# jsh58/Genrich

Measured on AMD Instinct MI355X. Metric: genome bases p-scored/sec, hg38 50M frags, higher is better.
Workload: dtype int32 pileup (1/120 units) + f64 p-values; 1 GPU; hg38 25 contigs (3088286401 bp), 50000000 paired fragments x 1 replicate(s), treatment only, -p 0.01 (BASELINE.json configs[1]); parallelism=chromosome-sharded x1, collectives=none, rccl_nranks=0, intervals=83948696, tables_written_in_step=none: the sweep walks the loose (end, V) slots, p = table p(V)

## Files before the change

genrich_amd/csrc/gx_api.hip:

```cpp
#include "gx_host_ctx.h"
#include "gx_host_coll.h"
#include "gx_host_build.h"
#include "gx_host_sweep.h"
#include "gx_host_stats.h"
#include "gx_host_count.h"
#include "gx_host_regions.h"



extern "C" {

const char* gx_strerror(int status) {
  switch (status) {
    case GX_OK: return "";
    case GX_ERR_MEM: return "Cannot allocate memory";
    case GX_ERR_GEN: return "No analyzable genome (length=0)";
    case GX_ERR_EXPT: return "Experimental sample has no analyzable fragments";
    case GX_ERR_PILE: return "Invalid pileup value (< 0)";
    case GX_ERR_POS: return ": read aligned beyond reference end";
    case GX_ERR_ALNS: return "Disallowed number of alignments";
    case GX_ERR_ARR: return "Failure creating experimental pileup";
    case GX_ERR_PVAL: return "Failure collecting p-values";
    case GX_ERR_DF: return "Invalid df in pchisq()";
    case GX_ERR_ORDER: return "API called out of order";
// ... 38 lines not shown
  memset(ctx->riskHost.p, 0, 32);
  HIPCHECK(hipMemsetAsync(ctx->dRisk.p, 0, 32, ctx->stream));
  HIPCHECK(hipMemsetAsync(ctx->dDeep.p, 0, sizeof(DeepTab), ctx->stream));
  HIPCHECK(hipMemsetAsync(ctx->misc.p, 0, M_WORDS * 4, ctx->stream));
  HIPCHECK(hipMemsetAsync(ctx->dScal.p, 0, sizeof(Scalars), ctx->stream));
  HIPCHECK(hipMemsetAsync(ctx->dStatus.p, 0, 64, ctx->stream));
  HIPCHECK(hipFuncSetAttribute(reinterpret_cast<const void*>(k_tile<true, false>),
                               hipFuncAttributeMaxDynamicSharedMemorySize, TL_LDS * 4));
  {
    hipDeviceProp_t prop;
    HIPCHECK(hipGetDeviceProperties(&prop, ctx->device));
    ctx->numCU = prop.multiProcessorCount;
    int nb = 0;
    HIPCHECK(hipOccupancyMaxActiveBlocksPerMultiprocessor(&nb, k_tile<true, false>, TL_NT, TL_LDS * 4));
    ctx->resTile = std::max(1, nb) * ctx->numCU;
    HIPCHECK(hipOccupancyMaxActiveBlocksPerMultiprocessor(&nb, k_tile<true, true>, TL_NT, TL_LDS_HALF * 4));
    ctx->resTileHalf = std::max(1, nb) * ctx->numCU;
    HIPCHECK(hipOccupancyMaxActiveBlocksPerMultiprocessor(&nb, k_tile_fast, 64, 0));
    ctx->resTileFast = std::max(1, std::min(nb, TF_WG_PER_CU)) * ctx->numCU;
    if (ctx->knob.debug)
      fprintf(stderr, "k_tile workgroups: half %d, wide %d, fast %d\n", ctx->resTileHalf, ctx->resTile, ctx->resTileFast);
    HIPCHECK(hipOccupancyMaxActiveBlocksPerMultiprocessor(&nb, k_scan_iv, STL_NT, 0));
    ctx->resSweep = std::max(1, std::min(nb, 4)) * ctx->numCU;
  }
  HIPCHECK(hipStreamSynchronize(ctx->stream));
  return GX_OK;
}

void gx_destroy(gx_ctx* ctx) {
  if (!ctx) return;
  (void)hipSetDevice(ctx->device);
  if (ctx->stream) (void)hipStreamSynchronize(ctx->stream);
  if (ctx->comm) {
    if (const gxrccl::Api* api = gxrccl::load(nullptr)) (void)api->commDestroy(ctx->comm);
    ctx->comm = nullptr;
  }
  for (auto& ph : ctx->phases) {
    (void)hipEventDestroy(ph.a);
    (void)hipEventDestroy(ph.b);
  }
  if (ctx->stream) (void)hipStreamDestroy(ctx->stream);
  if (ctx->side) (void)hipStreamDestroy(ctx->side);
  if (ctx->sideEv) (void)hipEventDestroy(ctx->sideEv);
  for (hipEvent_t e : ctx->evPool) (void)hipEventDestroy(e);
  for (hipEvent_t e : ctx->stageFree) if (e) (void)hipEventDestroy(e);
  delete ctx;
// ... 745 lines not shown
```

genrich_amd/csrc/gx_host_build.h:

```cpp
#pragma once
namespace {

uint64_t genome_len_for(const gx_ctx* ctx, const std::vector<uint8_t>& present) {
  uint64_t g = 0;
  for (u32 i = 0; i < ctx->nChrom; i++)
    if (!ctx->skip[i] && present[i]) {
      g += ctx->len[i];
      for (size_t j = 0; j + 1 < ctx->bed[i].size(); j += 2) g -= ctx->bed[i][j + 1] - ctx->bed[i][j];
    }
  return g;
}

int upload_chroms(gx_ctx* ctx, bool force = true) {
  bool changed = force;
  for (u32 i = 0; i < ctx->nChrom; i++) {
    const u32 f = (ctx->skip[i] ? CH_SKIP : 0) | (ctx->save[i] ? CH_SAVE : 0) | (ctx->owned[i] ? CH_OWNED : 0);
    changed |= f != ctx->hChrom[i].flags;
    ctx->hChrom[i].flags = f;
  }
  if (!changed) return GX_OK;
  HIPCHECK(hipMemcpyAsync(ctx->dChrom.p, ctx->hChrom.data(), ctx->nChrom * sizeof(DChrom), hipMemcpyHostToDevice,
                          ctx->stream));
  return GX_OK;
}
// ... 11 lines not shown
  return GX_OK;
}

int flush_begin(gx_ctx* ctx) {
  if (!ctx->beginPending) return GX_OK;
  hipLaunchKernelGGL(k_begin_sample, dim3(1), dim3(64), 0, ctx->stream, ctx->dScal.as<Scalars>(), ctx->beginGenome);
  ctx->beginPending = false;
  return GX_OK;
}

int stash_or_pack(gx_ctx* ctx, Pileup& P) {
  if (ctx->hasBed) return pack_pileup(ctx, P);
  if (P.inLoose) return GX_OK;
  recycle(ctx, P.looseEnd);
  recycle(ctx, P.looseV);
  recycle(ctx, P.meta);
  P.looseEnd = std::move(ctx->looseEnd);
  P.looseV = std::move(ctx->looseV);
  P.meta = std::move(ctx->tileMeta);
  P.inLoose = true;
  return GX_OK;
}

template <typename Segs> static u32 class_chunks(const Segs& segs) {
  u32 best = 0;
  for (u32 x = 0; x < (u32)NXCD; x++) {
    u32 c = 0;
    for (auto& sg : segs) {
      const u32 b = (u32)((sg.n + S2_CHUNK - 1) / S2_CHUNK);
      c += b / NXCD + (b % NXCD > x ? 1u : 0u);
    }
    best = std::max(best, c);
  }
  return best;
}

int unpack_segs(gx_ctx* ctx, bool all) {
  size_t total = 0;
  auto wanted = [&](const gx_ctx::Seg& sg) {
    return sg.packed && sg.n && (all || (reinterpret_cast<uintptr_t>(sg.p) & 15u) || (!sg.ready && (sg.n & 1u)));
  };
  for (auto& sg : ctx->segs)
    if (wanted(sg)) total += sg.n;
  if (!total) return GX_OK;
  if (ctx->unpackUsed == ctx->unpackBufs.size()) ctx->unpackBufs.emplace_back();
  DevBuf& buf = ctx->unpackBufs[ctx->unpackUsed++];
  HIPCHECK(buf.ensure(total * sizeof(gx_event)));
  hipStream_t s = ctx->stream;
  gx_event* at = buf.as<gx_event>();
  for (auto& sg : ctx->segs) {
    if (!wanted(sg)) continue;
    if (sg.ready) HIPCHECK(hipStreamWaitEvent(s, sg.ready, 0));
    hipLaunchKernelGGL(k_unpack_events, dim3((u32)std::min<size_t>((sg.n + 255) / 256, 8192)), dim3(256), 0, s,
                       reinterpret_cast<const uint2*>(sg.p), sg.n, reinterpret_cast<uint4*>(at));
    sg.p = at;
    sg.ready = nullptr;
    sg.packed = false;
// ... 26 lines not shown
  const bool pairsAllowed = !K.noPairs;
  const bool fracOk = pairsAllowed && !K.noFracPairs;
  const bool fracLikely = ctx->sawFrac || ctx->fracHint;
  const bool fused = P.fused =
      !backoff && unit32 && (!ctx->hasBed || (pairsAllowed && !K.noBedFused && !fracLikely)) && ctx->sbShift <= SBT_MAXSHIFT && !noFused &&
      (!fracLikely || fracOk) && !ctx->fusedOff && !forceSlowFrag && (size_t)nEv <= (size_t)std::max(1u, nL1base) * 64000 &&
      (size_t)2 * nEv + nTiles + ctx->nBedEdges + 64 < ((size_t)1 << 30);
  P.pairs = fused && !reuseSort && pairsAllowed;
  P.fracPairs = P.pairs && fracLikely;
  int sbS = ctx->sbShift;
  u32 nL1 = nL1base;
  const bool forceHalf = K.forceHalfBins != 0;
  if (P.pairs && (!P.fracPairs || forceHalf || K.fracHalfBins) && sbS > 0 &&
      (forceHalf || (size_t)2 * nEv > (size_t)std::max(1u, nL1base) * (SBT_KEYCAP - SBT_KEYCAP / 10)) &&
      ((nTiles + (1u << (sbS - 1)) - 1) >> (sbS - 1)) <= (u32)MAX_BINS_P && !K.noHalfBins) {
    sbS--;
    nL1 = (nTiles + (1u << sbS) - 1) >> sbS;
  }
  P.sbS = sbS, P.nL1 = nL1;
  P.jmax = ctx->ptJmax;
  P.poolPages[0] = P.poolPages[1] = (u32)(nEv >> PgCfg<u32>::SHIFT) + NXCD * nL1 + 4;
  P.poolPages[2] = (u32)(((size_t)2 * nEv) >> PgCfg<u64>::SHIFT) + NXCD * nL1 + 4;
  P.nCoarse = (std::max(1u, nL1) + (1u << s2_fine_shift(nL1)) - 1) >> s2_fine_shift(nL1);
  P.jmaxC = class_chunks(ctx->segs) + 3;
  for (auto& sg : ctx->segs) P.nWG1 += (u32)((sg.n + S2_CHUNK - 1) / S2_CHUNK);
  P.wantEarly = !isCtrl && (!P.multiRank || P.earlyColl) && !ctx->par.qval_opt && !ctx->hasBed && unit32 && !noLoose && !forceSlowFrag &&
                !ctx->sawFrac;
  const bool qLooseMay = ctx->par.qval_opt && !K.noQLoose && !ctx->qLooseBad && !ctx->sawFrac && !ctx->fracHint && !K.noPackHist;
  P.wantLate = !P.wantEarly && !isCtrl && !P.multiRank && (!ctx->par.qval_opt || qLooseMay) && !ctx->hasBed && unit32 && !noLoose &&
               !K.noLateLoose && fused && !forceSlowFrag;
  P.closeInScan = P.wantEarly && !P.multiRank;
  P.looseCap = (size_t)2 * nEv + nTiles + ctx->nBedEdges + 16;
  P.ivCap = (size_t)2 * nEv + ctx->nChrom + ctx->nBedEdges + 16;
  P.tChunks = (nTiles + STL_CHUNK - 1) / STL_CHUNK;
  P.fragFused = !ctx->hasBed && (!fused || P.fracPairs);
  P.dense = P.pairs && (size_t)2 * nEv > (size_t)std::max(1u, nL1) * (SBT_KEYCAP - SBT_KEYCAP / 16);
  if (P.dense) {
    const size_t want = (size_t)2 * nEv / std::max(1u, nL1);
    auto rounds = [&](u32 tr) { return (want + sbt_keycap(tr) - 1) / sbt_keycap(tr); };
    P.denseSmall = rounds((u32)SBT_TR_DENSE) < rounds((u32)SBT_TR);
    if (K.sbtTr) P.denseSmall = K.sbtTr == SBT_TR_DENSE;
  }
  return GX_OK;
}

PagedStream paged(const gx_ctx* ctx, const BuildPlan& P, int q) {
  const gx_ctx::Stream& st = ctx->str[q];
// ... 89 lines not shown
  HIPCHECK(hipMemsetAsync(ctx->looseCtl.p, 0, ctx->looseCtl.cap, s));
  HIPCHECK(hipMemsetAsync(&ctx->fragSum.as<FragFix>()->nList, 0, 12, s));
  HIPCHECK(hipMemsetAsync(nw_word(ctx, NW_WIDE), 0, 4, s));
  HIPCHECK(hipMemsetAsync(nw_word(ctx, NW_HEAVY), 0, 4, s));
  return GX_OK;
}

int sort_level1(gx_ctx* ctx, const BuildPlan& P) {
  hipStream_t s = ctx->stream;
  FragFix* ff = ctx->fragSum.as<FragFix>();
  if ((ctx->hasBed && !P.fused) || !P.unit32 || ctx->knob.forceSlowFrag) HIPCHECK(hipMemsetAsync(&ff->slow, 1, 4, s));
  if (P.reuseSort) return dbg_sync(ctx, "k_sort1");
  const PagedStream PG0 = paged(ctx, P, 0), PG1 = paged(ctx, P, 1), PG2 = paged(ctx, P, 2);
  const Sort1Out so1{ff->fragSum, &ff->slow, ctx->endAtLen.as<u32>(), nw_word(ctx, NW_HOT)};
  const u32 nListsC = NXCD * P.nCoarse;
  const PagedStream PC{ctx->poolC.p, ctx->ptC.as<u32>(), ctx->curC.as<u32>(), ctx->curC.as<u32>() + nListsC, P.jmaxC, P.nWG1 + 2 * nListsC + 8, nListsC};
  static constexpr decltype(&k_sort_a<false, false>) SORT_A[2][2] = {{k_sort_a<false, false>, k_sort_a<false, true>},
                                                                     {k_sort_a<true, false>, k_sort_a<true, true>}};
  for (auto& seg : ctx->segs) {
    if (!seg.n) continue;
    if (seg.ready) HIPCHECK(hipStreamWaitEvent(s, seg.ready, 0));
    const u32 blocks = (u32)((seg.n + S1_CHUNK - 1) / S1_CHUNK);
    if (P.pairs) {
      hipLaunchKernelGGL(SORT_A[P.fracPairs][seg.packed], dim3(blocks), dim3(S2_NT), 0, s, seg.p, (u32)seg.n, ctx->dChrom.as<DChrom>(), ctx->nChrom, P.sbS,
                         P.nL1, P.nCoarse, PC, ctx->auxC.as<uint8_t>(), PG2, ctx->binNet.as<int>(), so1, ctx->dStatus.as<u32>());
      ctx->packedUsed |= seg.packed;
    } else
      hipLaunchKernelGGL(P.unit32 ? k_sort1<true> : k_sort1<false>, dim3(blocks), dim3(S1_NT), 0, s, seg.p, (u32)seg.n,
                         ctx->dChrom.as<DChrom>(), ctx->nChrom, P.sbS, P.nL1, PG0, PG1, PG2, so1, ctx->dStatus.as<u32>());
  }
  if (P.pairs && P.nEv)
    hipLaunchKernelGGL(k_sort_b, dim3(NXCD * (P.jmaxC - 3 + P.nCoarse)), dim3(S2_NT), 0, s, PC, (const uint8_t*)ctx->auxC.as<uint8_t>(),
                       P.nCoarse, P.nL1, PG0, ctx->dStatus.as<u32>());
  return dbg_sync(ctx, "k_sort1");
}

long long* early_words(const gx_ctx* ctx, const BuildPlan& P) { return P.earlyColl ? ctx->dColl.as<long long>() + 4 : nullptr; }
int early_allreduce(gx_ctx* ctx, const BuildPlan& P) {
  if (!P.earlyColl) return GX_OK;
  hipLaunchKernelGGL(k_early_words, dim3(1), dim3(64), 0, ctx->stream, ctx->fragSum.as<FragFix>(), P.wantEarly ? 0 : 1, early_words(ctx, P));
  if (int rc__ = allreduce_words(ctx, early_words(ctx, P), 3)) return rc__;
  ctx->earlyOwed = false;
  return GX_OK;
}

int scan_bins(gx_ctx* ctx, const BuildPlan& P) {
  gx_ctx::Stream* S = ctx->str;
  auto capOf = [&](int shift) -> u32 { return P.jmax >= (1u << (31 - shift)) ? 0x7FFFFFFFu : P.jmax << shift; };
  BinScan bs{{S[0].cursor.as<u32>(), S[1].cursor.as<u32>(), S[2].cursor.as<u32>()},
             {capOf(PgCfg<u32>::SHIFT), capOf(PgCfg<u32>::SHIFT), capOf(PgCfg<u64>::SHIFT)},
             {S[0].sbOff.as<u32>(), S[1].sbOff.as<u32>(), S[2].sbOff.as<u32>()},
             ctx->endAtLen.as<u32>(), ctx->chromW0.as<int>(), ctx->nChrom, ctx->fragSum.as<FragFix>(), ctx->dScal.as<Scalars>(), ctx->looseCtl.as<LooseCtl>(),
             P.wantEarly ? 1 : 0, P.pairs ? 1 : 0, ctx->binNet.as<int>(), nw_word(ctx, NW_NEED_PAGES), early_words(ctx, P)};
  static_assert(PV_LUT % 1024 == 0, "k_bins_lut: four of k_pval_lut's workgroups per block");
  if (P.wantEarly)
    hipLaunchKernelGGL(k_bins_lut, dim3(4 + PV_LUT / 1024), dim3(1024), 0, ctx->stream, bs, P.nL1, ctx->pvLut.as<float>(),
// ... 429 lines not shown
```

genrich_amd/csrc/gx_host_ctx.h:

```cpp
#pragma once
#include <hip/hip_runtime.h>
#include <rocprim/device/device_radix_sort.hpp>

#include <algorithm>
#include <cmath>
#include <cstdio>
#include <cstdlib>
#include <cstring>
#include <atomic>
#include <chrono>
#include <string>
#include <vector>
#include <unistd.h>

#include "gx_merge.h"
#include "gx_rccl.h"
#include "gx_sort.h"
#include "gx_tile_fast.h"
#include "gx_sbtile.h"
#include "gx_dups.h"
#include "gx_bhx.h"
#include "gx_saturate.h"
#include "gx_count.h"
#include "gx_regions.h"
// ... 119 lines not shown
  int noFracPairs = 0;
  int noBedFused = 0;
  int bhVariant = -1;
  int mergeWg = 0;
  int noQLoose = 0;
  int noLateLoose = 0;
  int noLazyQ = 0;
  int noPackHist = 0;
  int noMergeP = 0;
  int forceHalfBins = 0;
  int noHalfBins = 0;
  int fracHalfBins = 0;
  int noEarlyColl = 0;
  int regWindows = 0;
  int noDenseBh = 0;
  int qtMulti = 0;
  int forceColl = 0;
  int sbShift = -1;
  long long runCapMin = 0;
  int bhCapLog = 0;
  int ptJmax = 0;
  int sbtTr = 0;
  int sbtGrid = 0;
  int roctx = 0;
  int fault = 0;
};
struct BuildPlan {
  int isCtrl = 0;
  bool reuseSort = false;
  u32 nEv = 0;
  bool unit32 = false;
  bool multiRank = false;
  bool earlyColl = false;
  bool fused = false;
  bool pairs = false;
  bool fracPairs = false;
  int sbS = 0;
  u32 nL1 = 0;
  u32 nCoarse = 0, jmaxC = 0, nWG1 = 0;
  u32 jmax = 0;
  u32 poolPages[3] = {0, 0, 0};
  bool wantEarly = false;
  bool wantLate = false;
  bool closeInScan = false;
  bool dense = false;
  bool denseSmall = false;
  bool fragFused = false;
  size_t looseCap = 0, ivCap = 0;
  u32 tChunks = 0;
  bool masks() const { return wantEarly || wantLate; }
};
struct KnobDef { const char* name; int Knobs::*i; long long Knobs::*ll; };
const KnobDef KNOBS[] = {
    {"GX_DEBUG", &Knobs::debug, nullptr}, {"GX_DEBUG_RETRY", &Knobs::debugRetry, nullptr}, {"GX_NO_SPIN", &Knobs::noSpin, nullptr},
    {"GX_FORCE_REC64", &Knobs::forceRec64, nullptr}, {"GX_FORCE_SLOWFRAG", &Knobs::forceSlowFrag, nullptr},
    {"GX_NO_FUSED", &Knobs::noFused, nullptr}, {"GX_NO_LOOSE", &Knobs::noLoose, nullptr}, {"GX_NO_PAIRS", &Knobs::noPairs, nullptr},
    {"GX_NO_FRAC_PAIRS", &Knobs::noFracPairs, nullptr}, {"GX_NO_BED_FUSED", &Knobs::noBedFused, nullptr}, {"GX_NO_MERGE_P", &Knobs::noMergeP, nullptr}, {"GX_NO_PACK_HIST", &Knobs::noPackHist, nullptr}, {"GX_NO_LAZY_Q", &Knobs::noLazyQ, nullptr}, {"GX_NO_LATE_LOOSE", &Knobs::noLateLoose, nullptr}, {"GX_NO_Q_LOOSE", &Knobs::noQLoose, nullptr}, {"GX_MERGE_WG", &Knobs::mergeWg, nullptr}, {"GX_BH_VARIANT", &Knobs::bhVariant, nullptr}, {"GX_FORCE_HALF_BINS", &Knobs::forceHalfBins, nullptr},
    {"GX_NO_HALF_BINS", &Knobs::noHalfBins, nullptr}, {"GX_FRAC_HALF_BINS", &Knobs::fracHalfBins, nullptr}, {"GX_NO_EARLY_COLL", &Knobs::noEarlyColl, nullptr},
    {"GX_NO_DENSE_BH", &Knobs::noDenseBh, nullptr}, {"GX_REG_WINDOWS", &Knobs::regWindows, nullptr}, {"GX_QT_MULTI", &Knobs::qtMulti, nullptr}, {"GX_FORCE_COLL", &Knobs::forceColl, nullptr},
    {"GX_SBSHIFT", &Knobs::sbShift, nullptr}, {"GX_RUN_CAP_MIN", nullptr, &Knobs::runCapMin}, {"GX_BH_CAPLOG", &Knobs::bhCapLog, nullptr},
    {"GX_PT_JMAX", &Knobs::ptJmax, nullptr}, {"GX_FAULT", &Knobs::fault, nullptr}, {"GX_SBT_TR", &Knobs::sbtTr, nullptr}, {"GX_SBT_GRID", &Knobs::sbtGrid, nullptr},
    {"GX_ROCTX", &Knobs::roctx, nullptr},
};
bool set_knob(Knobs& k, const char* name, const char* value) {
  for (const KnobDef& d : KNOBS)
    if (!strcmp(d.name, name)) {
      long long v = 1;
      if (value && *value) {
        char* end = nullptr;
        v = strtoll(value, &end, 10);
        if (end == value) v = 1;
      }
      if (d.i) k.*(d.i) = (int)v; else k.*(d.ll) = v;
      return true;
    }
  return false;
}

}

struct gx_ctx {
  gx_params par{};
  Knobs knob;
  int device = 0;
// ... 92 lines not shown
  PinnedBuf hPeaks;
  size_t nHostPeaks = 0;
  u32* nIvTarget = nullptr;
  PinnedBuf mailBuf;
  HostMail* mail = nullptr;
  uint64_t genomeLenUsed = 0, peakBP = 0;
  int rank = 0, world = 1;
  gx_allreduce_i64_fn allreduce = nullptr;
  void* user = nullptr;
  ncclComm_t comm = nullptr;
  bool forceColl = false;
  DevBuf bigBins;
  DevBuf dColl, dCounts, dGather, bhDense, bhxSmall, bhxRecv, bhxKeys, bhxLens, bhxQ, bhxOut, bhxAns;
  bool rangeBhUsed = false;
  bool denseBhUsed = false;
  int phaseLevel = 0;
  std::string phaseFilter = "tile";
  u32 mailSeq = 0;
  u32 statusSeen = 1;
  u64 runCap = 0, runSeen = 0;
  bool phaseOpen = false;
  bool roctxOpen = false;
  int numCU = 0, resTile = 0, resTileHalf = 0, resTileFast = 0, resSweep = 0;
  std::vector<DevBuf> pool;
  struct KeptSample {
    int rep = 0;
    bool ctrl = false;
    std::vector<Seg> segs;
    std::vector<uint8_t> save;
    std::vector<DevBuf> chunks, unpacks;
    DevBuf sat;
  };
  bool countOn = false;
  bool peaksReady = false;
  bool countsReady = false;
  std::vector<KeptSample> kept;
  u32 cntPk = 0;
  DevBuf cntIn, cntIdx, cntDiff, cntRes;
  PinnedBuf cntStage, cntHost;
  bool cntLdsSet = false;
  bool regionsReady = false;
  size_t regN = 0;
  u32 regSamples = 0;
  u32 regInvCap = 1u << 14;
  DevBuf regIn, regIdx, regHist, regSums, regRes, regInv;
  PinnedBuf regStage, regHost;
// ... 236 lines not shown
```

genrich_amd/csrc/gx_sort.h:

```cpp
#pragma once
#include "gx_kernels.h"
#include "gx_stats.h"

namespace gx {

constexpr u32 ST_PT_FULL = 512u;
constexpr u32 ST_SB_FULL = 1024u;
constexpr u32 ST_SB_FRAC = 2048u;

template <typename R> struct PgCfg { static constexpr int SHIFT = 12; };
template <> struct PgCfg<u32> { static constexpr int SHIFT = 13; };
constexpr u32 PG_BYTES = 32768;

struct PagedStream {
  void* pool;
  u32* pt;
  u32* cursor;
  u32* pagesUsed;
  u32 jmax, poolPages;
  u32 nLists;
};

__device__ __forceinline__ u32 first_page(u32 list) { return 1u + list; }

// ... 479 lines not shown
#define GX_S2_BATCH 4
#endif
constexpr int S2_BATCH = GX_S2_BATCH;
constexpr int S2_LCHROM = 96;
constexpr int S2_ITEMS = 8192 / S2_NT;
static_assert(S2_ITEMS == 16 || S2_ITEMS == 8, "512 or 1024 threads");
constexpr int S2_CHUNK = S2_NT * S2_ITEMS;
constexpr int S2_KEYS = 128;
constexpr int MAX_BINS_P = 8192;
__host__ __device__ inline int s2_fine_shift(u32 nBins) { return nBins > 4096u ? 7 : 6; }
static_assert(S2_CHUNK == (1 << PgCfg<u32>::SHIFT), "k_sort_b: one workgroup per page of a coarse list");
static_assert(S2_CHUNK == S1_CHUNK, "one grid size for the level-1 kernels");

struct S2Lds {
  u32 cnt[S2_KEYS];
  __attribute__((aligned(16))) uint4 run[S2_KEYS];
  u32 total;
  u32 wtot[2];
  u32 scratch[24];
  u32 stage[S2_CHUNK];
  uint16_t ka[S2_CHUNK];
};

template <bool AUX, int KEYS>
__device__ __forceinline__ void scatter64(const u32 (&rec)[S2_ITEMS], u32 (&ka)[S2_ITEMS], const PagedStream& P,
                                          uint8_t* __restrict__ auxPool, u32 listBase, u32 nKeys, S2Lds& L, u32* __restrict__ st) {
  static_assert(KEYS == 64 || KEYS == 128, "one or two owner wavefronts");
  constexpr int SHIFT = PgCfg<u32>::SHIFT;
  constexpr u32 PG = 1u << SHIFT;
  constexpr u32 KM = (u32)KEYS - 1u;
#pragma unroll
  for (int k = 0; k < S2_ITEMS; k++) ka[k] = (ka[k] & 0xFFFFu) | ((rec[k] != NULL32 ? atomicAdd(&L.cnt[ka[k] & KM], 1u) : 0u) << 16);
  __syncthreads();
  const bool owner = threadIdx.x < (u32)KEYS;
  const u32 key = threadIdx.x;
  u32 c = 0, o = 0, inc = 0, li = 0;
  if (owner) {
    c = key < nKeys ? L.cnt[key] : 0u;
    li = listBase + key;
    if (c) o = atomicAdd(&P.cursor[li], c);
    inc = (u32)dpp_scan_add((int)c);
    if ((key & 63u) == 63u) L.wtot[key >> 6] = inc;
  }
  if (KEYS == 64 && threadIdx.x == 0) L.wtot[1] = 0;
  __syncthreads();
  const u32 in0 = o & (PG - 1), j0 = o >> SHIFT, j1 = (o + c - 1) >> SHIFT;
  u32* row = P.pt + (size_t)li * P.jmax;
  u32 p0 = 0, p1 = 0;
  bool wait0 = false;
  if (owner) {
    if (key == 0) L.total = L.wtot[0] + L.wtot[1];
    if (c) {
      if (j1 != j0) p1 = page_alloc(P, row, j1, st);
      if (j0 == 0)
        p0 = first_page(li);
      else if (in0 == 0)
        p0 = page_alloc(P, row, j0, st);
      else
        wait0 = true;
    }
  }
  __syncthreads();
  if (owner) {
    if (wait0) p0 = page_wait(P, row, j0, st);
    L.run[key] = make_uint4(inc - c + (key >= 64u ? L.wtot[0] : 0u), min(c, PG - in0), (p0 << SHIFT) + in0, p1 << SHIFT);
  }
  __syncthreads();
#pragma unroll
  for (int k = 0; k < S2_ITEMS; k++)
    if (rec[k] != NULL32) {
      const u32 pos = L.run[ka[k] & KM].x + (ka[k] >> 16);
      L.stage[pos] = rec[k];
      L.ka[pos] = (uint16_t)ka[k];
    }
  __syncthreads();
  u32* pool = reinterpret_cast<u32*>(P.pool);
  const u32 cnt = L.total;
#pragma unroll
  for (int h = 0; h < S2_ITEMS; h += 8) {
    u32 v[8], kk[8];
#pragma unroll
    for (int k = 0; k < 8; k++) {
      const u32 i = (u32)(h + k) * S2_NT + threadIdx.x, ii = i < cnt ? i : 0u;
      v[k] = L.stage[ii];
      kk[k] = L.ka[ii];
    }
#pragma unroll
    for (int k = 0; k < 8; k++) {
      const u32 i = (u32)(h + k) * S2_NT + threadIdx.x;
      const uint4 rn = L.run[kk[k] & KM];
      const u32 r = i - rn.x;
      const u32 dst = r < rn.y ? rn.z + r : rn.w + (r - rn.y);
      if (i < cnt) {
        pool[dst] = v[k];
        if (AUX) auxPool[dst] = (uint8_t)(kk[k] >> 8);
      }
    }
  }
}

__device__ __forceinline__ uint4 unpack_event8(u32 start, u32 lcc) {
  return make_uint4(lcc >> 19, start, start + (lcc & 0xFFFFu), (0xA8654321u >> (4u * ((lcc >> 16) & 7u))) & 15u);
}
__global__ __launch_bounds__(256) void k_unpack_events(const uint2* __restrict__ in, size_t n, uint4* __restrict__ out) {
  for (size_t i = (size_t)blockIdx.x * 256 + threadIdx.x; i < n; i += (size_t)gridDim.x * 256) {
    const uint2 e = in[i];
    out[i] = unpack_event8(e.x, e.y);
  }
}

template <bool FRAC, bool PACKED = false>
__global__ __launch_bounds__(S2_NT, GX_S2A_WAVES) void k_sort_a(const gx_event* __restrict__ ev, u32 n, const DChrom* __restrict__ chroms,
                                                     u32 nChrom, int sbShift, u32 nBins, u32 nCoarse, PagedStream PC,
                                                     uint8_t* __restrict__ auxPool, PagedStream PF, int* __restrict__ binNet,
                                                     Sort1Out out, u32* __restrict__ st) {
  __shared__ S2Lds L;
  __shared__ DChrom lchrom[S2_LCHROM];
  const int fineShift = s2_fine_shift(nBins);
  if (!FRAC && (__hip_atomic_load(st, __ATOMIC_RELAXED, __HIP_MEMORY_SCOPE_AGENT) & ST_SB_FRAC)) return;
  const bool chromLds = nChrom <= (u32)S2_LCHROM;
  const u32 x = blockIdx.x % NXCD;
  const u32 begin = blockIdx.x * S2_CHUNK;
  const u32 binMask = (1u << sbShift) - 1u;
  u32 bad = 0, slow = 0, fracSeen = 0;
  u32 covered32 = 0;
  u32 rec[S2_ITEMS], ka[S2_ITEMS];
  if (threadIdx.x < S2_KEYS) L.cnt[threadIdx.x] = 0;
  const uint4* __restrict__ evb = reinterpret_cast<const uint4*>(ev) + begin;
  const u32 lastIn = n - 1u - begin;
#pragma unroll
  for (int k0 = 0; k0 < S2_ITEMS; k0 += S2_BATCH) {
    uint4 e[S2_BATCH];
    bool have[S2_BATCH];
    if constexpr (PACKED) {
      static_assert(S2_BATCH % 2 == 0, "two packed events per 16-byte load");
      const uint4* __restrict__ evp = reinterpret_cast<const uint4*>(reinterpret_cast<const uint2*>(ev) + begin);
#pragma unroll
      for (int q = 0; q < S2_BATCH; q += 2) {
        const u32 lp = ((k0 + q) >> 1) * S2_NT + threadIdx.x;
        have[q] = 2u * lp <= lastIn;
        have[q + 1] = 2u * lp + 1u <= lastIn;
        const uint4 two = evp[min(lp, lastIn >> 1)];
        e[q] = unpack_event8(two.x, two.y);
        e[q + 1] = unpack_event8(two.z, two.w);
      }
    } else {
#pragma unroll
    for (int q = 0; q < S2_BATCH; q++) {
      const u32 li = (k0 + q) * S2_NT + threadIdx.x;
      have[q] = li <= lastIn;
      e[q] = evb[min(li, lastIn)];
    }
    }
    if (k0 == 0) {
      if (chromLds)
        for (u32 i = threadIdx.x; i < nChrom; i += S2_NT) lchrom[i] = chroms[i];
      __syncthreads();
    }
    DChrom cq[S2_BATCH];
    if (chromLds) {
#pragma unroll
      for (int q = 0; q < S2_BATCH; q++) cq[q] = lchrom[min(e[q].x, nChrom - 1)];
    } else {
#pragma unroll
      for (int q = 0; q < S2_BATCH; q++) cq[q] = chroms[min(e[q].x, nChrom - 1)];
    }
#pragma unroll
    for (int q = 0; q < S2_BATCH; q++) {
      const DChrom c = cq[q];
      const u32 cnt = e[q].w;
      const bool cntOk = FRAC ? (cnt <= 10u && ((0x57Eu >> cnt) & 1u)) : cnt == 1u;
      const bool ok1 = have[q] && cntOk && e[q].x < nChrom;
      const bool act = chrom_active(c);
      const u32 len = e[q].z - e[q].y;
      const u32 t0 = c.tileBase + (e[q].y >> TB), t1 = c.tileBase + (e[q].z >> TB);
      const u32 bin = t0 >> sbShift;
      constexpr u32 LENB = FRAC ? 9u : PAIR_LEN_BITS;
      const bool fast = ok1 && act && e[q].z < c.len && len - 1u < (1u << LENB) - 1u && e[q].y < e[q].z && (t1 >> sbShift) == bin;
      const bool nothing = !have[q] || (ok1 && !act);
      const u32 cls = FRAC ? (u32)((0x70605432100ull >> (4u * (cnt & 15u))) & 7ull) << 9 : 0u;
      fracSeen |= (u32)(FRAC && fast && cnt != 1u);
      rec[k0 + q] = fast ? ((((t0 & binMask) << TB) | (e[q].y & (TILE - 1))) << PAIR_LEN_BITS) | cls | len : NULL32;
      ka[k0 + q] = (bin >> fineShift) | ((bin & ((1u << fineShift) - 1u)) << 8);
      covered32 += fast && cnt == 1u ? len : 0u;
      slow |= (u32)(!fast && !nothing) << (k0 + q);
    }
    __builtin_amdgcn_sched_barrier(0);
  }
  u64 covered = covered32;
  scatter64<true, 64>(rec, ka, PC, auxPool, x * nCoarse, nCoarse, L, st);
  if (__ballot(slow != 0)) {
#pragma unroll 1
    for (int k = 0; k < S2_ITEMS; k++) {
      bool mine = (slow >> k) & 1u;
      if (!__ballot(mine)) continue;
      u64 r0 = 0, r1 = 0;
      u32 l0 = 0, l1 = 0;
      bool h1 = false;
      if (mine) {
        uint4 e;
        if constexpr (PACKED) {
          const uint2 e8 = reinterpret_cast<const uint2*>(ev)[begin + 2u * ((u32)(k >> 1) * S2_NT + threadIdx.x) + (u32)(k & 1)];
          e = unpack_event8(e8.x, e8.y);
        } else
          e = reinterpret_cast<const uint4*>(ev)[begin + k * S2_NT + threadIdx.x];
        const Endpoints p = convert_event<true>(e, chroms[min(e.x, nChrom - 1)], true, nChrom, out, bad, covered);
        mine = p.w != 0;
        if (mine) {
          if (p.w != GX_UNIT) {
            atomicOr(out.slowFrag, FRAG_SLOW_FRAC);
            if (!FRAC) {
              atomicOr(st, ST_SB_FRAC);
              mine = false;
            }
          }
          if (mine) {
          r0 = make_rec64(p.t0, p.o0, p.w);
          l0 = x * nBins + (p.t0 >> sbShift);
          atomicAdd(&binNet[p.t0 >> sbShift], p.w);
          h1 = p.t1 != NULL_TILE;
          }
        }
        if (h1) {
          r1 = make_rec64(p.t1, p.o1, -p.w);
          l1 = x * nBins + (p.t1 >> sbShift);
          atomicAdd(&binNet[p.t1 >> sbShift], -p.w);
        }
      }
      append_single(PF, l0, r0, mine, st);
      append_single(PF, l1, r1, h1, st);
    }
  }
  if (bad) atomicOr(st, bad);
  if (FRAC && __ballot(fracSeen != 0) && lane_id() == 0) atomicOr(out.slowFrag, FRAG_SLOW_FRAC);
  covered = wave_sum(covered);
  if (lane_id() == 0 && covered) atomicAdd(&out.fragSum[(blockIdx.x * 8 + (threadIdx.x >> 6)) % FRAG_SLOTS], covered);
}

__global__ __launch_bounds__(S2_NT, GX_S2B_WAVES) void k_sort_b(PagedStream PC, const uint8_t* __restrict__ auxPool, u32 nCoarse, u32 nBins,
                                                     PagedStream PP, u32* __restrict__ st) {
  constexpr int SHIFT = PgCfg<u32>::SHIFT;
  __shared__ S2Lds L;
  __shared__ u32 sList, sPage, sCount;
  if (threadIdx.x < 64) {
    const u32 xc = blockIdx.x % NXCD, q = blockIdx.x / NXCD;
    const u32 len = threadIdx.x < nCoarse ? PC.cursor[xc * nCoarse + threadIdx.x] : 0u;
    const u32 np = (len + S2_CHUNK - 1) >> SHIFT;
    const u32 inc = (u32)dpp_scan_add((int)np), ex = inc - np;
    if (threadIdx.x == 0) sCount = 0;
    L.cnt[threadIdx.x] = 0;
    L.cnt[threadIdx.x + 64] = 0;
    __builtin_amdgcn_wave_barrier();
    if (q >= ex && q < inc) {
      const u32 j = q - ex;
      sList = xc * nCoarse + threadIdx.x;
      sPage = j;
      sCount = min((u32)S2_CHUNK, len - (j << SHIFT));
    }
  }
  __syncthreads();
  const u32 count = sCount;
  if (count == 0) return;
  const u32 li = sList, j = sPage;
  const u32 x = li / nCoarse, cb = li - x * nCoarse;
  const u32 page = j ? __hip_atomic_load(&PC.pt[(size_t)li * PC.jmax + j], __ATOMIC_RELAXED, __HIP_MEMORY_SCOPE_AGENT) - 1u : first_page(li);
  const u32* src = reinterpret_cast<const u32*>(PC.pool) + ((size_t)page << SHIFT);
  const uint8_t* srcA = auxPool + ((size_t)page << SHIFT);
  u32 rec[S2_ITEMS], ka[S2_ITEMS];
  {
    constexpr int NQ = S2_ITEMS / 4;
    uint4 r4[NQ];
#pragma unroll
    for (int q = 0; q < NQ; q++) r4[q] = reinterpret_cast<const uint4*>(src)[threadIdx.x * NQ + q];
    u32 aw[4] = {0u, 0u, 0u, 0u};
    if (NQ == 4) {
      const uint4 a4 = reinterpret_cast<const uint4*>(srcA)[threadIdx.x];
      aw[0] = a4.x; aw[1] = a4.y; aw[2] = a4.z; aw[3] = a4.w;
    } else {
      const uint2 a2 = reinterpret_cast<const uint2*>(srcA)[threadIdx.x];
      aw[0] = a2.x; aw[1] = a2.y;
    }
#pragma unroll
    for (int q = 0; q < NQ; q++) {
      const u32 rw[4] = {r4[q].x, r4[q].y, r4[q].z, r4[q].w};
#pragma unroll
      for (int j = 0; j < 4; j++) {
        const u32 i = threadIdx.x * S2_ITEMS + q * 4 + j;
        rec[q * 4 + j] = i < count ? rw[j] : NULL32;
        ka[q * 4 + j] = (aw[q] >> (8 * j)) & 0xFFu;
      }
    }
  }
  const int fineShift = s2_fine_shift(nBins);
  const u32 firstBin = cb << fineShift, nk = min(1u << fineShift, nBins - firstBin);
  if (fineShift == 7)
    scatter64<false, 128>(rec, ka, PP, nullptr, x * nBins + firstBin, nk, L, st);
  else
    scatter64<false, 64>(rec, ka, PP, nullptr, x * nBins + firstBin, nk, L, st);
}

struct BinScan {
  const u32* cursor[3];
  u32 cap[3];
  u32* sbOff[3];
  const u32* endAtLen;
  int* chromW0;
  u32 nChrom;
  const FragFix* ff;
  Scalars* scal;
  LooseCtl* ctl;
  int wantEarly;
  int pairMode;
  const int* binNet;
  u32* needPages;
  const long long* early;
};

__device__ __forceinline__ void scan_bins_body(const BinScan& B, u32 nBins, u32 block, u32* __restrict__ scratch, u32* ready) {
  if (block == 3) {
    if (threadIdx.x < 64 && B.wantEarly) {
      static_assert(FRAG_SLOTS <= 64, "one lane per partial sum");
// ... 342 lines not shown
```

Measured before the change: 2728 Gbases/s.

## Make pair sort kernels persistent with cross-chunk prefetch of events and pages

k_sort_a and k_sort_b become grid-stride persistent kernels, each sized from occupancy to a whole multiple of the XCD count. k_sort_a keeps a register ring of prefetched event batches that reaches into the next chunk, so global loads overlap the convert and scatter work. It also hoists the chromosome table load and the early-exit check out of the per-chunk path. k_sort_b prefetches the next page while scattering the current one. scatter64 now clears its LDS counters itself so they can be reused across iterations, and the page-table capacity bound is recomputed for the new grid.

```diff
diff --git a/genrich_amd/csrc/gx_api.hip b/genrich_amd/csrc/gx_api.hip
--- a/genrich_amd/csrc/gx_api.hip
+++ b/genrich_amd/csrc/gx_api.hip
@@ -84,6 +84,16 @@
       fprintf(stderr, "k_tile workgroups: half %d, wide %d, fast %d\n", ctx->resTileHalf, ctx->resTile, ctx->resTileFast);
     HIPCHECK(hipOccupancyMaxActiveBlocksPerMultiprocessor(&nb, k_scan_iv, STL_NT, 0));
     ctx->resSweep = std::max(1, std::min(nb, 4)) * ctx->numCU;
+    int nbA = 1 << 30;
+    for (auto k : {k_sort_a<false, false>, k_sort_a<false, true>, k_sort_a<true, false>, k_sort_a<true, true>}) {
+      HIPCHECK(hipOccupancyMaxActiveBlocksPerMultiprocessor(&nb, k, S2_NT, 0));
+      nbA = std::min(nbA, nb);
+    }
+    auto wholeXcds = [](int g) { return g > NXCD ? g - g % NXCD : std::max(1, g); };
+    ctx->resSortA = wholeXcds(std::max(1, nbA) * ctx->numCU);
+    HIPCHECK(hipOccupancyMaxActiveBlocksPerMultiprocessor(&nb, k_sort_b, S2_NT, 0));
+    ctx->resSortB = wholeXcds(std::max(1, nb) * ctx->numCU);
+    if (ctx->knob.debug) fprintf(stderr, "pair sort workgroups: k_sort_a %d, k_sort_b %d\n", ctx->resSortA, ctx->resSortB);
   }
   HIPCHECK(hipStreamSynchronize(ctx->stream));
   return GX_OK;
diff --git a/genrich_amd/csrc/gx_host_build.h b/genrich_amd/csrc/gx_host_build.h
--- a/genrich_amd/csrc/gx_host_build.h
+++ b/genrich_amd/csrc/gx_host_build.h
@@ -57,17 +57,17 @@
   return GX_OK;
 }
 
-template <typename Segs> static u32 class_chunks(const Segs& segs) {
-  u32 best = 0;
-  for (u32 x = 0; x < (u32)NXCD; x++) {
-    u32 c = 0;
-    for (auto& sg : segs) {
-      const u32 b = (u32)((sg.n + S2_CHUNK - 1) / S2_CHUNK);
-      c += b / NXCD + (b % NXCD > x ? 1u : 0u);
-    }
-    best = std::max(best, c);
-  }
-  return best;
+static u32 sort_a_grid(const gx_ctx* ctx, u32 chunks) {
+  const u32 g = ctx->knob.s2Grid > 0 ? (u32)ctx->knob.s2Grid : (u32)std::max(1, ctx->resSortA);
+  return std::max(1u, std::min(chunks, g));
+}
+static u32 class_chunks(const gx_ctx* ctx) {
+  u32 perClass[NXCD] = {};
+  for (auto& sg : ctx->segs) {
+    const u32 b = (u32)((sg.n + S2_CHUNK - 1) / S2_CHUNK), g = sort_a_grid(ctx, b);
+    for (u32 w = 0; w < g && w < b; w++) perClass[w % NXCD] += (b - w + g - 1) / g;
+  }
+  return *std::max_element(perClass, perClass + NXCD);
 }
 
 int unpack_segs(gx_ctx* ctx, bool all) {
@@ -140,7 +140,7 @@
   P.poolPages[0] = P.poolPages[1] = (u32)(nEv >> PgCfg<u32>::SHIFT) + NXCD * nL1 + 4;
   P.poolPages[2] = (u32)(((size_t)2 * nEv) >> PgCfg<u64>::SHIFT) + NXCD * nL1 + 4;
   P.nCoarse = (std::max(1u, nL1) + (1u << s2_fine_shift(nL1)) - 1) >> s2_fine_shift(nL1);
-  P.jmaxC = class_chunks(ctx->segs) + 3;
+  P.jmaxC = class_chunks(ctx) + 3;
   for (auto& sg : ctx->segs) P.nWG1 += (u32)((sg.n + S2_CHUNK - 1) / S2_CHUNK);
   P.wantEarly = !isCtrl && (!P.multiRank || P.earlyColl) && !ctx->par.qval_opt && !ctx->hasBed && unit32 && !noLoose && !forceSlowFrag &&
                 !ctx->sawFrac;
@@ -276,16 +276,19 @@
     if (seg.ready) HIPCHECK(hipStreamWaitEvent(s, seg.ready, 0));
     const u32 blocks = (u32)((seg.n + S1_CHUNK - 1) / S1_CHUNK);
     if (P.pairs) {
-      hipLaunchKernelGGL(SORT_A[P.fracPairs][seg.packed], dim3(blocks), dim3(S2_NT), 0, s, seg.p, (u32)seg.n, ctx->dChrom.as<DChrom>(), ctx->nChrom, P.sbS,
+      hipLaunchKernelGGL(SORT_A[P.fracPairs][seg.packed], dim3(sort_a_grid(ctx, blocks)), dim3(S2_NT), 0, s, seg.p, (u32)seg.n, ctx->dChrom.as<DChrom>(), ctx->nChrom, P.sbS,
                          P.nL1, P.nCoarse, PC, ctx->auxC.as<uint8_t>(), PG2, ctx->binNet.as<int>(), so1, ctx->dStatus.as<u32>());
       ctx->packedUsed |= seg.packed;
     } else
       hipLaunchKernelGGL(P.unit32 ? k_sort1<true> : k_sort1<false>, dim3(blocks), dim3(S1_NT), 0, s, seg.p, (u32)seg.n,
                          ctx->dChrom.as<DChrom>(), ctx->nChrom, P.sbS, P.nL1, PG0, PG1, PG2, so1, ctx->dStatus.as<u32>());
   }
-  if (P.pairs && P.nEv)
-    hipLaunchKernelGGL(k_sort_b, dim3(NXCD * (P.jmaxC - 3 + P.nCoarse)), dim3(S2_NT), 0, s, PC, (const uint8_t*)ctx->auxC.as<uint8_t>(),
+  if (P.pairs && P.nEv) {
+    const u32 want = ctx->knob.s2Grid > 0 ? (u32)ctx->knob.s2Grid : (u32)std::max(1, ctx->resSortB);
+    const u32 gridB = std::min((u32)NXCD * (P.jmaxC - 3 + P.nCoarse), (want + NXCD - 1) / NXCD * NXCD);
+    hipLaunchKernelGGL(k_sort_b, dim3(gridB), dim3(S2_NT), 0, s, PC, (const uint8_t*)ctx->auxC.as<uint8_t>(),
                        P.nCoarse, P.nL1, PG0, ctx->dStatus.as<u32>());
+  }
   return dbg_sync(ctx, "k_sort1");
 }
 
diff --git a/genrich_amd/csrc/gx_host_ctx.h b/genrich_amd/csrc/gx_host_ctx.h
--- a/genrich_amd/csrc/gx_host_ctx.h
+++ b/genrich_amd/csrc/gx_host_ctx.h
@@ -165,6 +165,7 @@
   int ptJmax = 0;
   int sbtTr = 0;
   int sbtGrid = 0;
+  int s2Grid = 0;
   int roctx = 0;
   int fault = 0;
 };
@@ -203,6 +204,7 @@
     {"GX_NO_DENSE_BH", &Knobs::noDenseBh, nullptr}, {"GX_REG_WINDOWS", &Knobs::regWindows, nullptr}, {"GX_QT_MULTI", &Knobs::qtMulti, nullptr}, {"GX_FORCE_COLL", &Knobs::forceColl, nullptr},
     {"GX_SBSHIFT", &Knobs::sbShift, nullptr}, {"GX_RUN_CAP_MIN", nullptr, &Knobs::runCapMin}, {"GX_BH_CAPLOG", &Knobs::bhCapLog, nullptr},
     {"GX_PT_JMAX", &Knobs::ptJmax, nullptr}, {"GX_FAULT", &Knobs::fault, nullptr}, {"GX_SBT_TR", &Knobs::sbtTr, nullptr}, {"GX_SBT_GRID", &Knobs::sbtGrid, nullptr},
+    {"GX_S2_GRID", &Knobs::s2Grid, nullptr},
     {"GX_ROCTX", &Knobs::roctx, nullptr},
 };
 bool set_knob(Knobs& k, const char* name, const char* value) {
@@ -341,6 +343,7 @@
   bool phaseOpen = false;
   bool roctxOpen = false;
   int numCU = 0, resTile = 0, resTileHalf = 0, resTileFast = 0, resSweep = 0;
+  int resSortA = 0, resSortB = 0;
   std::vector<DevBuf> pool;
   struct KeptSample {
     int rep = 0;
diff --git a/genrich_amd/csrc/gx_sort.h b/genrich_amd/csrc/gx_sort.h
--- a/genrich_amd/csrc/gx_sort.h
+++ b/genrich_amd/csrc/gx_sort.h
@@ -1,4 +1,5 @@
 #pragma once
+#include <type_traits>
 #include "gx_kernels.h"
 #include "gx_stats.h"
 
@@ -525,6 +526,12 @@
   uint16_t ka[S2_CHUNK];
 };
 
+__device__ __forceinline__ u32 fresh_tid() {
+  u32 t = threadIdx.x;
+  asm volatile("" : "+v"(t));
+  return t;
+}
+
 template <bool AUX, int KEYS>
 __device__ __forceinline__ void scatter64(const u32 (&rec)[S2_ITEMS], u32 (&ka)[S2_ITEMS], const PagedStream& P,
                                           uint8_t* __restrict__ auxPool, u32 listBase, u32 nKeys, S2Lds& L, u32* __restrict__ st) {
@@ -532,20 +539,22 @@
   constexpr int SHIFT = PgCfg<u32>::SHIFT;
   constexpr u32 PG = 1u << SHIFT;
   constexpr u32 KM = (u32)KEYS - 1u;
+  const u32 tid = fresh_tid();
 #pragma unroll
   for (int k = 0; k < S2_ITEMS; k++) ka[k] = (ka[k] & 0xFFFFu) | ((rec[k] != NULL32 ? atomicAdd(&L.cnt[ka[k] & KM], 1u) : 0u) << 16);
   __syncthreads();
-  const bool owner = threadIdx.x < (u32)KEYS;
-  const u32 key = threadIdx.x;
+  const bool owner = tid < (u32)KEYS;
+  const u32 key = tid;
   u32 c = 0, o = 0, inc = 0, li = 0;
   if (owner) {
     c = key < nKeys ? L.cnt[key] : 0u;
+    L.cnt[key] = 0;
     li = listBase + key;
     if (c) o = atomicAdd(&P.cursor[li], c);
     inc = (u32)dpp_scan_add((int)c);
     if ((key & 63u) == 63u) L.wtot[key >> 6] = inc;
   }
-  if (KEYS == 64 && threadIdx.x == 0) L.wtot[1] = 0;
+  if (KEYS == 64 && tid == 0) L.wtot[1] = 0;
   __syncthreads();
   const u32 in0 = o & (PG - 1), j0 = o >> SHIFT, j1 = (o + c - 1) >> SHIFT;
   u32* row = P.pt + (size_t)li * P.jmax;
@@ -579,18 +588,19 @@
   __syncthreads();
   u32* pool = reinterpret_cast<u32*>(P.pool);
   const u32 cnt = L.total;
-#pragma unroll
-  for (int h = 0; h < S2_ITEMS; h += 8) {
-    u32 v[8], kk[8];
-#pragma unroll
-    for (int k = 0; k < 8; k++) {
-      const u32 i = (u32)(h + k) * S2_NT + threadIdx.x, ii = i < cnt ? i : 0u;
+  constexpr int SB = 8;
+#pragma unroll
+  for (int h = 0; h < S2_ITEMS; h += SB) {
+    u32 v[SB], kk[SB];
+#pragma unroll
+    for (int k = 0; k < SB; k++) {
+      const u32 i = (u32)(h + k) * S2_NT + tid, ii = i < cnt ? i : 0u;
       v[k] = L.stage[ii];
       kk[k] = L.ka[ii];
     }
 #pragma unroll
-    for (int k = 0; k < 8; k++) {
-      const u32 i = (u32)(h + k) * S2_NT + threadIdx.x;
+    for (int k = 0; k < SB; k++) {
+      const u32 i = (u32)(h + k) * S2_NT + tid;
       const uint4 rn = L.run[kk[k] & KM];
       const u32 r = i - rn.x;
       const u32 dst = r < rn.y ? rn.z + r : rn.w + (r - rn.y);
@@ -612,6 +622,9 @@
   }
 }
 
+#ifndef GX_S2_PFL
+#define GX_S2_PFL 4
+#endif
 template <bool FRAC, bool PACKED = false>
 __global__ __launch_bounds__(S2_NT, GX_S2A_WAVES) void k_sort_a(const gx_event* __restrict__ ev, u32 n, const DChrom* __restrict__ chroms,
                                                      u32 nChrom, int sbShift, u32 nBins, u32 nCoarse, PagedStream PC,
@@ -619,54 +632,79 @@
                                                      Sort1Out out, u32* __restrict__ st) {
   __shared__ S2Lds L;
   __shared__ DChrom lchrom[S2_LCHROM];
+  __shared__ u32 sStop[3];
   const int fineShift = s2_fine_shift(nBins);
-  if (!FRAC && (__hip_atomic_load(st, __ATOMIC_RELAXED, __HIP_MEMORY_SCOPE_AGENT) & ST_SB_FRAC)) return;
   const bool chromLds = nChrom <= (u32)S2_LCHROM;
   const u32 x = blockIdx.x % NXCD;
-  const u32 begin = blockIdx.x * S2_CHUNK;
+  const u32 nChunks = (n + S2_CHUNK - 1) / S2_CHUNK;
   const u32 binMask = (1u << sbShift) - 1u;
-  u32 bad = 0, slow = 0, fracSeen = 0;
+  u32 bad = 0, fracSeen = 0;
+  u64 covered = 0;
+  constexpr int NL = PACKED ? S2_BATCH / 2 : S2_BATCH;
+  constexpr int NB = S2_ITEMS / S2_BATCH, PFB = GX_S2_PFL / NL;
+  static_assert(S2_BATCH % 2 == 0, "two packed events per 16-byte load");
+  static_assert(PFB >= 1 && NB % PFB == 0, "a batch's place in the ring is the same in every chunk");
+  auto load_batch = [&](u32 tid, u32 begin, int k0, uint4 (&raw)[NL]) {
+    const u32 lastIn = n - 1u - begin;
+    if constexpr (PACKED) {
+      const uint4* __restrict__ evp = reinterpret_cast<const uint4*>(reinterpret_cast<const uint2*>(ev) + begin);
+#pragma unroll
+      for (int q = 0; q < NL; q++) raw[q] = evp[min(((u32)(k0 >> 1) + q) * S2_NT + tid, lastIn >> 1)];
+    } else {
+      const uint4* __restrict__ evb = reinterpret_cast<const uint4*>(ev) + begin;
+#pragma unroll
+      for (int q = 0; q < NL; q++) raw[q] = evb[min((u32)(k0 + q) * S2_NT + tid, lastIn)];
+    }
+  };
+  u32 sv = 0;
+  if (!FRAC && threadIdx.x == 0) sv = __hip_atomic_load(st, __ATOMIC_RELAXED, __HIP_MEMORY_SCOPE_AGENT);
+  if (threadIdx.x < S2_KEYS) L.cnt[threadIdx.x] = 0;
+  uint4 ring[PFB][NL];
+#pragma unroll
+  for (int b = 0; b < PFB; b++) load_batch(threadIdx.x, blockIdx.x * S2_CHUNK, b * S2_BATCH, ring[b]);
+  if (chromLds)
+    for (u32 i = threadIdx.x; i < nChrom; i += S2_NT) lchrom[i] = chroms[i];
+  if (!FRAC && threadIdx.x == 0) sStop[2] = sv & ST_SB_FRAC;
+  __syncthreads();
+  if (!FRAC && sStop[2]) return;
+  auto chunks = [&](auto inLds) {
+  constexpr bool CLDS = decltype(inLds)::value;
+  u32 it = 0;
+  for (u32 chunk = blockIdx.x; chunk < nChunks; chunk += gridDim.x, it++) {
+  const u32 tid = fresh_tid();
+  const u32 begin = chunk * S2_CHUNK;
+  const u32 lastIn = n - 1u - begin;
+  u32 slow = 0;
   u32 covered32 = 0;
   u32 rec[S2_ITEMS], ka[S2_ITEMS];
-  if (threadIdx.x < S2_KEYS) L.cnt[threadIdx.x] = 0;
-  const uint4* __restrict__ evb = reinterpret_cast<const uint4*>(ev) + begin;
-  const u32 lastIn = n - 1u - begin;
+  const u32 next = chunk + gridDim.x;
 #pragma unroll
   for (int k0 = 0; k0 < S2_ITEMS; k0 += S2_BATCH) {
+    asm volatile("" ::: "memory");
+    uint4 (&raw)[NL] = ring[(k0 / S2_BATCH) % PFB];
     uint4 e[S2_BATCH];
     bool have[S2_BATCH];
     if constexpr (PACKED) {
-      static_assert(S2_BATCH % 2 == 0, "two packed events per 16-byte load");
-      const uint4* __restrict__ evp = reinterpret_cast<const uint4*>(reinterpret_cast<const uint2*>(ev) + begin);
 #pragma unroll
       for (int q = 0; q < S2_BATCH; q += 2) {
-        const u32 lp = ((k0 + q) >> 1) * S2_NT + threadIdx.x;
+        const u32 lp = ((k0 + q) >> 1) * S2_NT + tid;
         have[q] = 2u * lp <= lastIn;
         have[q + 1] = 2u * lp + 1u <= lastIn;
-        const uint4 two = evp[min(lp, lastIn >> 1)];
-        e[q] = unpack_event8(two.x, two.y);
-        e[q + 1] = unpack_event8(two.z, two.w);
+        e[q] = unpack_event8(raw[q >> 1].x, raw[q >> 1].y);
+        e[q + 1] = unpack_event8(raw[q >> 1].z, raw[q >> 1].w);
       }
     } else {
 #pragma unroll
+      for (int q = 0; q < S2_BATCH; q++) {
+        have[q] = (k0 + q) * S2_NT + tid <= lastIn;
+        e[q] = raw[q];
+      }
+    }
+    DChrom cq[S2_BATCH];
+#pragma unroll
     for (int q = 0; q < S2_BATCH; q++) {
-      const u32 li = (k0 + q) * S2_NT + threadIdx.x;
-      have[q] = li <= lastIn;
-      e[q] = evb[min(li, lastIn)];
-    }
-    }
-    if (k0 == 0) {
-      if (chromLds)
-        for (u32 i = threadIdx.x; i < nChrom; i += S2_NT) lchrom[i] = chroms[i];
-      __syncthreads();
-    }
-    DChrom cq[S2_BATCH];
-    if (chromLds) {
-#pragma unroll
-      for (int q = 0; q < S2_BATCH; q++) cq[q] = lchrom[min(e[q].x, nChrom - 1)];
-    } else {
-#pragma unroll
-      for (int q = 0; q < S2_BATCH; q++) cq[q] = chroms[min(e[q].x, nChrom - 1)];
+      if constexpr (CLDS) cq[q] = lchrom[min(e[q].x, nChrom - 1)];
+      else cq[q] = chroms[min(e[q].x, nChrom - 1)];
     }
 #pragma unroll
     for (int q = 0; q < S2_BATCH; q++) {
@@ -688,9 +726,16 @@
       covered32 += fast && cnt == 1u ? len : 0u;
       slow |= (u32)(!fast && !nothing) << (k0 + q);
     }
+#pragma unroll
+    for (int q = 0; q < S2_BATCH; q++) asm volatile("" : "+v"(rec[k0 + q]), "+v"(ka[k0 + q]));
+    asm volatile("" : "+v"(slow), "+v"(covered32), "+v"(fracSeen));
+    if (k0 / S2_BATCH + PFB < NB)
+      load_batch(tid, begin, k0 + PFB * S2_BATCH, raw);
+    else if (next < nChunks)
+      load_batch(tid, next * S2_CHUNK, k0 + PFB * S2_BATCH - S2_ITEMS, raw);
     __builtin_amdgcn_sched_barrier(0);
   }
-  u64 covered = covered32;
+  covered += covered32;
   scatter64<true, 64>(rec, ka, PC, auxPool, x * nCoarse, nCoarse, L, st);
   if (__ballot(slow != 0)) {
 #pragma unroll 1
@@ -703,10 +748,10 @@
       if (mine) {
         uint4 e;
         if constexpr (PACKED) {
-          const uint2 e8 = reinterpret_cast<const uint2*>(ev)[begin + 2u * ((u32)(k >> 1) * S2_NT + threadIdx.x) + (u32)(k & 1)];
+          const uint2 e8 = reinterpret_cast<const uint2*>(ev)[begin + 2u * ((u32)(k >> 1) * S2_NT + tid) + (u32)(k & 1)];
           e = unpack_event8(e8.x, e8.y);
         } else
-          e = reinterpret_cast<const uint4*>(ev)[begin + k * S2_NT + threadIdx.x];
+          e = reinterpret_cast<const uint4*>(ev)[begin + k * S2_NT + tid];
         const Endpoints p = convert_event<true>(e, chroms[min(e.x, nChrom - 1)], true, nChrom, out, bad, covered);
         mine = p.w != 0;
         if (mine) {
@@ -734,6 +779,13 @@
       append_single(PF, l1, r1, h1, st);
     }
   }
+  if (!FRAC) {
+    if (tid == 0) sStop[it & 1u] = __hip_atomic_load(st, __ATOMIC_RELAXED, __HIP_MEMORY_SCOPE_AGENT) & ST_SB_FRAC;
+    if (it && sStop[(it - 1u) & 1u]) break;
+  }
+  }
+  };
+  if (chromLds) chunks(std::true_type{}); else chunks(std::false_type{});
   if (bad) atomicOr(st, bad);
   if (FRAC && __ballot(fracSeen != 0) && lane_id() == 0) atomicOr(out.slowFrag, FRAG_SLOW_FRAC);
   covered = wave_sum(covered);
@@ -743,63 +795,74 @@
 __global__ __launch_bounds__(S2_NT, GX_S2B_WAVES) void k_sort_b(PagedStream PC, const uint8_t* __restrict__ auxPool, u32 nCoarse, u32 nBins,
                                                      PagedStream PP, u32* __restrict__ st) {
   constexpr int SHIFT = PgCfg<u32>::SHIFT;
+  constexpr int NQ = S2_ITEMS / 4;
   __shared__ S2Lds L;
-  __shared__ u32 sList, sPage, sCount;
-  if (threadIdx.x < 64) {
-    const u32 xc = blockIdx.x % NXCD, q = blockIdx.x / NXCD;
-    const u32 len = threadIdx.x < nCoarse ? PC.cursor[xc * nCoarse + threadIdx.x] : 0u;
-    const u32 np = (len + S2_CHUNK - 1) >> SHIFT;
-    const u32 inc = (u32)dpp_scan_add((int)np), ex = inc - np;
-    if (threadIdx.x == 0) sCount = 0;
-    L.cnt[threadIdx.x] = 0;
-    L.cnt[threadIdx.x + 64] = 0;
-    __builtin_amdgcn_wave_barrier();
-    if (q >= ex && q < inc) {
-      const u32 j = q - ex;
-      sList = xc * nCoarse + threadIdx.x;
-      sPage = j;
-      sCount = min((u32)S2_CHUNK, len - (j << SHIFT));
-    }
-  }
-  __syncthreads();
-  const u32 count = sCount;
-  if (count == 0) return;
-  const u32 li = sList, j = sPage;
-  const u32 x = li / nCoarse, cb = li - x * nCoarse;
-  const u32 page = j ? __hip_atomic_load(&PC.pt[(size_t)li * PC.jmax + j], __ATOMIC_RELAXED, __HIP_MEMORY_SCOPE_AGENT) - 1u : first_page(li);
-  const u32* src = reinterpret_cast<const u32*>(PC.pool) + ((size_t)page << SHIFT);
-  const uint8_t* srcA = auxPool + ((size_t)page << SHIFT);
-  u32 rec[S2_ITEMS], ka[S2_ITEMS];
-  {
-    constexpr int NQ = S2_ITEMS / 4;
-    uint4 r4[NQ];
-#pragma unroll
-    for (int q = 0; q < NQ; q++) r4[q] = reinterpret_cast<const uint4*>(src)[threadIdx.x * NQ + q];
-    u32 aw[4] = {0u, 0u, 0u, 0u};
-    if (NQ == 4) {
-      const uint4 a4 = reinterpret_cast<const uint4*>(srcA)[threadIdx.x];
-      aw[0] = a4.x; aw[1] = a4.y; aw[2] = a4.z; aw[3] = a4.w;
-    } else {
-      const uint2 a2 = reinterpret_cast<const uint2*>(srcA)[threadIdx.x];
-      aw[0] = a2.x; aw[1] = a2.y;
-    }
-#pragma unroll
-    for (int q = 0; q < NQ; q++) {
-      const u32 rw[4] = {r4[q].x, r4[q].y, r4[q].z, r4[q].w};
-#pragma unroll
-      for (int j = 0; j < 4; j++) {
-        const u32 i = threadIdx.x * S2_ITEMS + q * 4 + j;
-        rec[q * 4 + j] = i < count ? rw[j] : NULL32;
-        ka[q * 4 + j] = (aw[q] >> (8 * j)) & 0xFFu;
-      }
-    }
-  }
+  const u32 xc = blockIdx.x % NXCD, stride = gridDim.x / NXCD;
+  const u32 lane = lane_id();
+  const u32 len = lane < nCoarse ? PC.cursor[xc * nCoarse + lane] : 0u;
+  const u32 np = (len + S2_CHUNK - 1) >> SHIFT;
+  const u32 inc = (u32)dpp_scan_add((int)np), ex = inc - np;
+  const u32 total = (u32)__builtin_amdgcn_readlane((int)inc, 63);
+  if (threadIdx.x < S2_KEYS) L.cnt[threadIdx.x] = 0;
+  __syncthreads();
+  struct Page { u32 cb, count, id; };
+  auto find = [&](u32 q) {
+    const int cb = __ffsll((unsigned long long)__ballot(q >= ex && q < inc)) - 1;
+    const u32 j = q - (u32)__builtin_amdgcn_readlane((int)ex, cb), li = xc * nCoarse + (u32)cb;
+    Page p;
+    p.cb = (u32)cb;
+    p.count = min((u32)S2_CHUNK, (u32)__builtin_amdgcn_readlane((int)len, cb) - (j << SHIFT));
+    p.id = j == 0 ? first_page(li) + 1u
+                  : j < PC.jmax ? max(1u, __hip_atomic_load(&PC.pt[(size_t)li * PC.jmax + j], __ATOMIC_RELAXED, __HIP_MEMORY_SCOPE_AGENT)) : 1u;
+    return p;
+  };
+  uint4 r4[NQ], a4 = make_uint4(0u, 0u, 0u, 0u);
+  auto load_page = [&](u32 tid, u32 id) {
+    const u32 page = id - 1u;
+    const u32* src = reinterpret_cast<const u32*>(PC.pool) + ((size_t)page << SHIFT);
+    const uint8_t* srcA = auxPool + ((size_t)page << SHIFT);
+#pragma unroll
+    for (int q = 0; q < NQ; q++) r4[q] = reinterpret_cast<const uint4*>(src)[tid * NQ + q];
+    if (NQ == 4)
+      a4 = reinterpret_cast<const uint4*>(srcA)[tid];
+    else {
+      const uint2 a2 = reinterpret_cast<const uint2*>(srcA)[tid];
+      a4.x = a2.x; a4.y = a2.y;
+    }
+  };
+  u32 q = blockIdx.x / NXCD;
+  if (q >= total) return;
+  Page cur = find(q), nxt = cur;
+  load_page(threadIdx.x, cur.id);
+  if (q + stride < total) nxt = find(q + stride);
   const int fineShift = s2_fine_shift(nBins);
-  const u32 firstBin = cb << fineShift, nk = min(1u << fineShift, nBins - firstBin);
-  if (fineShift == 7)
-    scatter64<false, 128>(rec, ka, PP, nullptr, x * nBins + firstBin, nk, L, st);
-  else
-    scatter64<false, 64>(rec, ka, PP, nullptr, x * nBins + firstBin, nk, L, st);
+  for (;;) {
+    const u32 tid = fresh_tid();
+    u32 rec[S2_ITEMS], ka[S2_ITEMS];
+    {
+      const u32 aw[4] = {a4.x, a4.y, a4.z, a4.w};
+#pragma unroll
+      for (int h = 0; h < NQ; h++) {
+        const u32 rw[4] = {r4[h].x, r4[h].y, r4[h].z, r4[h].w};
+#pragma unroll
+        for (int j = 0; j < 4; j++) {
+          const u32 i = tid * S2_ITEMS + h * 4 + j;
+          rec[h * 4 + j] = i < cur.count ? rw[j] : NULL32;
+          ka[h * 4 + j] = (aw[h] >> (8 * j)) & 0xFFu;
+        }
+      }
+    }
+    const u32 firstBin = cur.cb << fineShift, nk = min(1u << fineShift, nBins - firstBin);
+    if (fineShift == 7)
+      scatter64<false, 128>(rec, ka, PP, nullptr, xc * nBins + firstBin, nk, L, st);
+    else
+      scatter64<false, 64>(rec, ka, PP, nullptr, xc * nBins + firstBin, nk, L, st);
+    q += stride;
+    if (q >= total) break;
+    cur = nxt;
+    load_page(tid, cur.id);
+    if (q + stride < total) nxt = find(q + stride);
+  }
 }
 
 struct BinScan {
```

Result: faster. 2810 Gbases/s (median of 6 runs) (+3.0%).
